# libmir/mir-optim

Measured on AMD Instinct MI355X. Metric: LM iterations/sec, higher is better.
Workload: dtype f64

## Files before the change

mir_optim_amd/csrc/workloads_device.h:

```cpp
#pragma once

#include <hip/hip_runtime.h>
#include <omp.h>

#include <cmath>
#include <cstddef>
#include <cstdint>
#include <cstdlib>
#include <type_traits>

namespace {


template <int N> __device__ inline int dpp_row_ror(int v) { return __builtin_amdgcn_update_dpp(0, v, 0x120 + N, 0xF, 0xF, false); }
template <int N> __device__ inline double dpp_row_ror(double v)
{
    return __hiloint2double(dpp_row_ror<N>(__double2hiint(v)), dpp_row_ror<N>(__double2loint(v)));
}
template <int N> __device__ inline float dpp_row_ror(float v) { return __int_as_float(dpp_row_ror<N>(__float_as_int(v))); }
template <typename T> __device__ inline T sum16(T v)
{
    v += dpp_row_ror<8>(v);
    v += dpp_row_ror<4>(v);
    v += dpp_row_ror<2>(v);
    v += dpp_row_ror<1>(v);
    return v;
}

template <int N, typename F, int I = 0> __device__ __forceinline__ void wl_static_for(F&& f)
{
    if constexpr (I < N) {
        f(std::integral_constant<int, I>{});
        wl_static_for<N, F, I + 1>(static_cast<F&&>(f));
    }
}

__device__ inline double lane_pair_swap(double v)
{
    const int lo = __builtin_amdgcn_mov_dpp(__double2loint(v), 0xB1, 0xF, 0xF, true);
    const int hi = __builtin_amdgcn_mov_dpp(__double2hiint(v), 0xB1, 0xF, 0xF, true);
    return __hiloint2double(hi, lo);
}

__device__ inline double dtanh(double x)
{
    const double ax = fabs(x);
    const double t = fmin(2.0 * ax, 40.0);
    const double kf = rint(t * 1.4426950408889634);
    double r = fma(kf, -6.93147180369123816490e-01, t);
    r = fma(kf, -1.90821492927058770002e-10, r);
    double p = 1.0 / 6227020800.0;
    p = fma(p, r, 1.0 / 479001600.0);
    p = fma(p, r, 1.0 / 39916800.0);
    p = fma(p, r, 1.0 / 3628800.0);
    p = fma(p, r, 1.0 / 362880.0);
    p = fma(p, r, 1.0 / 40320.0);
    p = fma(p, r, 1.0 / 5040.0);
    p = fma(p, r, 1.0 / 720.0);
    p = fma(p, r, 1.0 / 120.0);
    p = fma(p, r, 1.0 / 24.0);
    p = fma(p, r, 1.0 / 6.0);
    p = fma(p, r, 0.5);
    p = fma(p, r, 1.0);
    p = fma(p, r, 1.0);
    const double e = ldexp(p, (int)kf);
    const double d = e + 1.0;
    double q = __builtin_amdgcn_rcp(d);
    q = fma(fma(-d, q, 1.0), q, q);
    q = fma(fma(-d, q, 1.0), q, q);
    return copysign(fma(-2.0, q, 1.0), x);
}
__device__ inline float dtanh(float v) { return tanhf(v); }
__device__ inline double dexp(double v) { return exp(v); }
__device__ inline float dexp(float v) { return expf(v); }


}
```

mir_optim_amd/csrc/workloads_gemm.hip:

```cpp
#include "workloads_gemm.h"
#include "workloads_device.h"

namespace {

template <int NK>
__global__ __launch_bounds__(1024) void k_tanh_linear_batched(const double* __restrict__ A, const double* __restrict__ b,
                                                               const double* __restrict__ X, double* __restrict__ Y,
                                                               size_t m, int n, int P)
{
    using Acc = __attribute__((ext_vector_type(4))) double;
    constexpr int NPAD = 4 * NK;
    constexpr int PITCH = NPAD + 2;
    __shared__ __attribute__((aligned(16))) double tile[2][16 * PITCH];
    const int tid = threadIdx.x, lane = tid & 63, wave = tid >> 6;
    const int fr = lane & 15, fq = lane >> 4;

    for (int idx = tid; idx < 2 * 16 * PITCH; idx += 1024) (&tile[0][0])[idx] = 0.0;
    __syncthreads();

    const int ppr = n / 2;
    const bool has_piece = tid < 16 * ppr;
    const int prow = has_piece ? tid / ppr : 0, pcol = has_piece ? tid % ppr : 0;
    const size_t ntiles = (m + 15) / 16;

    for (int pbase = 0; pbase < P; pbase += 256) {
        const int pl = pbase + wave * 16 + fr;
        const bool pok = pl < P;
        const bool wave_active = pbase + wave * 16 < P;
        double xf[NK];
#pragma unroll
        for (int s = 0; s < NK; ++s) {
            const int col = 4 * s + fq;
            xf[s] = (pok && col < n) ? X[(size_t)pl * n + col] : 0.0;
        }
        double2 stage = make_double2(0.0, 0.0);
        auto gload = [&](size_t t) {
            const size_t row = t * 16 + prow;
            if (has_piece && row < m) stage = *reinterpret_cast<const double2*>(A + row * (size_t)n + 2 * pcol);
            else stage = make_double2(0.0, 0.0);
        };
        auto lstore = [&](int buf) {
            if (has_piece) *reinterpret_cast<double2*>(&tile[buf][prow * PITCH + 2 * pcol]) = stage;
        };
        size_t t = blockIdx.x;
        if (t < ntiles) { gload(t); lstore(0); }
        if (t + gridDim.x < ntiles) gload(t + gridDim.x);
        __syncthreads();
        int buf = 0;
        Acc prev = {0.0, 0.0, 0.0, 0.0};
        size_t tprev = ntiles;
        auto epilogue = [&](const Acc& acc, size_t tt) {
#pragma unroll
            for (int r = 0; r < 4; ++r) {
                const size_t row = tt * 16 + fq + 4 * r;
                if (pok && tt < ntiles && row < m) Y[(size_t)pl * m + row] = dtanh(acc[r]) - b[row];
            }
        };
        for (; t < ntiles; t += gridDim.x) {
            if (wave_active) {
                Acc acc = {0.0, 0.0, 0.0, 0.0};
                const double* tp = &tile[buf][fr * PITCH + fq];
#pragma unroll
                for (int s = 0; s < NK; ++s) acc = __builtin_amdgcn_mfma_f64_16x16x4f64(tp[4 * s], xf[s], acc, 0, 0, 0);
                epilogue(prev, tprev);
                prev = acc;
                tprev = t;
            }
            if (t + gridDim.x < ntiles) lstore(buf ^ 1);
            if (t + 2 * (size_t)gridDim.x < ntiles) gload(t + 2 * (size_t)gridDim.x);
            __syncthreads();
            buf ^= 1;
        }
        if (wave_active) epilogue(prev, tprev);
        __syncthreads();
    }
}


typedef __attribute__((address_space(3))) void* wl_lds_ptr;
typedef const __attribute__((address_space(1))) void* wl_gbl_ptr;

__device__ __forceinline__ constexpr int tlb_rho(int i) { return ((i >> 2) >> 1) * 8 + 2 * (i & 3) + ((i >> 2) & 1); }
__device__ __forceinline__ constexpr int tlb_sigma(int i) { return (i + 12) & 15; }

template <int NK> struct TlbCfg {
    static constexpr int N = 4 * NK;
    static constexpr int PPR = N / 2;
    static constexpr int TILES = NK <= 32 ? 2 : 1;
    static constexpr bool SELF = NK > 32;
    static constexpr int COMPUTE_WAVES = 8, LOADER_WAVES = SELF ? 0 : 2;
    static constexpr int CHUNK = 16 * COMPUTE_WAVES;
    static constexpr int ROWS = 16 * TILES;
    static constexpr int STAGE_BYTES = ROWS * N * 8;
    static constexpr int IPS = STAGE_BYTES / 1024;
    static constexpr int NS = 4, D = 2, NSB = 8;
    static constexpr int B_OFF = NS * STAGE_BYTES;
    static constexpr int LDS_BYTES = B_OFF + NSB * 256;
    static constexpr int THREADS = 64 * (COMPUTE_WAVES + LOADER_WAVES);
    static constexpr bool FORK = NK == 32;
    static constexpr int NPRE = NK / 2 - 1;
    static constexpr int PRE_STAGE = TILES * NPRE * 16 * 8;
    static constexpr int PRE_OFF = LDS_BYTES;
    static constexpr int VOTE_OFF = PRE_OFF + 2 * PRE_STAGE;
    static constexpr int FORK_LDS_BYTES = VOTE_OFF + 16;
};

template <int NK, int LOADER>
__device__ __forceinline__ void tlb_issue(const double* __restrict__ A, const double* __restrict__ b, size_t m,
                                          unsigned char* smem, int lane, size_t S, size_t f)
{
    using C = TlbCfg<NK>;
    constexpr int MYI = C::IPS / 2;
    const unsigned char* Ab = reinterpret_cast<const unsigned char*>(A);
    const unsigned char* bb = reinterpret_cast<const unsigned char*>(b);
    const size_t stage = blockIdx.x + (f % S) * (size_t)gridDim.x;
    const size_t row0 = stage * C::ROWS;
    unsigned char* slot = smem + (f % C::NS) * C::STAGE_BYTES;
#pragma unroll
    for (int k = 0; k < MYI; ++k) {
        const int ins = LOADER + 2 * k;
        const int g = ins * 64 + lane;
        const int R = g / C::PPR, sp = g % C::PPR;
        size_t row = row0 + (R & 16) + tlb_rho(R & 15);
        row = row < m ? row : m - 1;
        const int piece = sp ^ tlb_sigma(R & 15);
        __builtin_amdgcn_global_load_lds((wl_gbl_ptr)(Ab + (row * C::N + 2 * piece) * 8),
                                         (wl_lds_ptr)(slot + ins * 1024), 16, 0, 2 );
    }
    if constexpr (LOADER == 1) {
        size_t row = row0 + (lane >> 1);
        row = row < m ? row : m - 1;
        __builtin_amdgcn_global_load_lds((wl_gbl_ptr)(bb + row * 8 + (lane & 1) * 4),
                                         (wl_lds_ptr)(smem + C::B_OFF + (f % C::NSB) * 256), 4, 0, 0);
    }
}

template <int NK, int LOADER>
__device__ __forceinline__ void tlb_loader(const double* __restrict__ A, const double* __restrict__ b, size_t m,
                                           unsigned char* smem, int lane, size_t S, size_t F)
{
    using C = TlbCfg<NK>;
    constexpr int OPS = C::IPS / 2 + (LOADER == 1 ? 1 : 0);
    auto issue = [&](size_t f) { tlb_issue<NK, LOADER>(A, b, m, smem, lane, S, f); };
    const size_t pre = F < (size_t)C::D ? F : (size_t)C::D;
    for (size_t f = 0; f < pre; ++f) issue(f);
    for (size_t f = 0; f < F; ++f) {
        if (f + C::D < F) {
            issue(f + C::D);
            asm volatile("s_waitcnt vmcnt(%0)" ::"n"(C::D * OPS) : "memory");
        } else {
            asm volatile("s_waitcnt vmcnt(0)" ::: "memory");
        }
        __builtin_amdgcn_s_barrier();
    }
}

template <int NK, bool ALIGNED, int GROUP, bool RM = false, bool DIFF = false>
__device__ __forceinline__ void tlb_compute(const double* __restrict__ A, const double* __restrict__ b,
                                            const double* __restrict__ X, double* __restrict__ Y, size_t m, int P,
                                            unsigned char* smem, int lane, int wave, size_t S, int nchunks)
{
    using C = TlbCfg<NK>;
    using Acc = __attribute__((ext_vector_type(4))) double;
    const int fr = lane & 15, fq = lane >> 4;
    const int v = fq ^ tlb_sigma(fr);
    int laddr[4];
#pragma unroll
    for (int k = 0; k < 4; ++k) laddr[k] = fr * C::N * 8 + ((4 * k) ^ v) * 16;

    constexpr int MYI = C::SELF ? C::IPS / C::COMPUTE_WAVES : 1;
    [[maybe_unused]] int roff[MYI], soff[MYI];
    [[maybe_unused]] unsigned is_next = 0, slot_next = 0, bslot_next = 0;
    [[maybe_unused]] const size_t Ftot = S * (size_t)nchunks;
    [[maybe_unused]] size_t fissued = 0;
    const unsigned char* Ab = reinterpret_cast<const unsigned char*>(A);
    const unsigned char* bb = reinterpret_cast<const unsigned char*>(b);
    if constexpr (C::SELF) {
#pragma unroll
        for (int k = 0; k < MYI; ++k) {
            const int g = (wave + C::COMPUTE_WAVES * k) * 64 + lane;
            const int R = g / C::PPR, sp = g % C::PPR;
            roff[k] = (R & 16) + tlb_rho(R & 15);
            soff[k] = 2 * (sp ^ tlb_sigma(R & 15)) * 8;
        }
    }
    auto issue = [&]() {
        const size_t row0 = (blockIdx.x + (size_t)is_next * gridDim.x) * C::ROWS;
        unsigned char* slot = smem + slot_next * C::STAGE_BYTES;
#pragma unroll
        for (int k = 0; k < MYI; ++k) {
            size_t row = row0 + roff[k];
            row = row < m ? row : m - 1;
            __builtin_amdgcn_global_load_lds((wl_gbl_ptr)(Ab + row * (C::N * 8) + soff[k]),
                                             (wl_lds_ptr)(slot + (wave + C::COMPUTE_WAVES * k) * 1024), 16, 0, 2 );
        }
        if (wave == 0) {
            size_t row = row0 + (lane >> 1);
            row = row < m ? row : m - 1;
            __builtin_amdgcn_global_load_lds((wl_gbl_ptr)(bb + row * 8 + (lane & 1) * 4),
                                             (wl_lds_ptr)(smem + C::B_OFF + bslot_next * 256), 4, 0, 0);
        }
        is_next = is_next + 1 == (unsigned)S ? 0 : is_next + 1;
        slot_next = (slot_next + 1) % C::NS;
        bslot_next = (bslot_next + 1) % C::NSB;
        ++fissued;
    };
    auto advance = [&]() {
        if constexpr (C::SELF) {
            if (fissued < Ftot) {
                issue();
                if (wave == 0) asm volatile("s_waitcnt vmcnt(%0)" ::"n"(C::D * (MYI + 1)) : "memory");
                else asm volatile("s_waitcnt vmcnt(%0)" ::"n"(C::D * MYI) : "memory");
            } else {
                asm volatile("s_waitcnt vmcnt(0)" ::: "memory");
            }
        }
    };
    if constexpr (C::SELF) {
        for (int d = 0; d < C::D && fissued < Ftot; ++d) issue();
        advance();
    }

    size_t f = 0;
    for (int ch = 0; ch < nchunks; ++ch) {
        const bool wave_active = ch * C::CHUNK + wave * 16 < P;
        if (!wave_active) {
            for (size_t s = 0; s < S; ++s) {
                __builtin_amdgcn_s_barrier();
                ++f;
                if (f < Ftot) advance();
            }
            continue;
        }
        int pl = ch * C::CHUNK + wave * 16 + fr;
        pl = pl < P ? pl : P - 1;
        double xf[NK];
#pragma unroll
        for (int s = 0; s < NK; ++s) xf[s] = X[(size_t)pl * C::N + 8 * (s >> 1) + 2 * fq + (s & 1)];
        double* yp = DIFF ? Y + (pl >> 1) : (RM ? Y + pl : Y + (size_t)pl * m);
        const size_t ldr = DIFF ? (size_t)(P >> 1) : (RM ? (size_t)P : 1);

        auto mfma_stage = [&](size_t ff, Acc& acc0, Acc& acc1) {
            const unsigned char* slot = smem + (ff % C::NS) * C::STAGE_BYTES;
            acc0 = Acc{0, 0, 0, 0};
            acc1 = Acc{0, 0, 0, 0};
            if constexpr (C::TILES == 2) {
#pragma unroll
                for (int j = 0; j < NK / 2; ++j) {
                    const int off = laddr[j & 3] + (j >> 2) * 256;
                    const double2 a0 = *reinterpret_cast<const double2*>(slot + off);
                    const double2 a1 = *reinterpret_cast<const double2*>(slot + off + 16 * C::N * 8);
                    acc0 = __builtin_amdgcn_mfma_f64_16x16x4f64(a0.x, xf[2 * j], acc0, 0, 0, 0);
                    acc1 = __builtin_amdgcn_mfma_f64_16x16x4f64(a1.x, xf[2 * j], acc1, 0, 0, 0);
                    acc0 = __builtin_amdgcn_mfma_f64_16x16x4f64(a0.y, xf[2 * j + 1], acc0, 0, 0, 0);
                    acc1 = __builtin_amdgcn_mfma_f64_16x16x4f64(a1.y, xf[2 * j + 1], acc1, 0, 0, 0);
                }
            } else {
#pragma unroll
                for (int j = 0; j < NK / 2; j += 2) {
                    const double2 a0 = *reinterpret_cast<const double2*>(slot + laddr[j & 3] + (j >> 2) * 256);
                    const double2 a1 = *reinterpret_cast<const double2*>(slot + laddr[(j + 1) & 3] + ((j + 1) >> 2) * 256);
                    acc0 = __builtin_amdgcn_mfma_f64_16x16x4f64(a0.x, xf[2 * j], acc0, 0, 0, 0);
                    acc1 = __builtin_amdgcn_mfma_f64_16x16x4f64(a1.x, xf[2 * j + 2], acc1, 0, 0, 0);
                    acc0 = __builtin_amdgcn_mfma_f64_16x16x4f64(a0.y, xf[2 * j + 1], acc0, 0, 0, 0);
                    acc1 = __builtin_amdgcn_mfma_f64_16x16x4f64(a1.y, xf[2 * j + 3], acc1, 0, 0, 0);
                }
                acc0 += acc1;
            }
        };
        auto epilogue_tile = [&](const Acc& acc, size_t row0, const unsigned char* bslot, auto full_tag) {
            constexpr bool FULL = decltype(full_tag)::value;
            const double2 b0 = *reinterpret_cast<const double2*>(bslot + 16 * fq);
            const double2 b1 = *reinterpret_cast<const double2*>(bslot + 64 + 16 * fq);
            const double y0 = dtanh(acc[0]) - b0.x, y1 = dtanh(acc[1]) - b0.y;
            const double y2 = dtanh(acc[2]) - b1.x, y3 = dtanh(acc[3]) - b1.y;
            const size_t ra = row0 + 2 * fq, rb = row0 + 8 + 2 * fq;
            if constexpr (DIFF) {
                const double d0 = y0 - lane_pair_swap(y0), d1 = y1 - lane_pair_swap(y1);
                const double d2 = y2 - lane_pair_swap(y2), d3 = y3 - lane_pair_swap(y3);
                if ((fr & 1) == 0) {
                    if (FULL || ra < m) yp[ra * ldr] = d0;
                    if (FULL || ra + 1 < m) yp[(ra + 1) * ldr] = d1;
                    if (FULL || rb < m) yp[rb * ldr] = d2;
                    if (FULL || rb + 1 < m) yp[(rb + 1) * ldr] = d3;
                }
            } else if constexpr (RM) {
                if (FULL || ra < m) yp[ra * ldr] = y0;
                if (FULL || ra + 1 < m) yp[(ra + 1) * ldr] = y1;
                if (FULL || rb < m) yp[rb * ldr] = y2;
                if (FULL || rb + 1 < m) yp[(rb + 1) * ldr] = y3;
            } else if constexpr (FULL && ALIGNED) {
                *reinterpret_cast<double2*>(yp + ra) = make_double2(y0, y1);
                *reinterpret_cast<double2*>(yp + rb) = make_double2(y2, y3);
            } else if constexpr (FULL) {
                yp[ra] = y0;
                yp[ra + 1] = y1;
                yp[rb] = y2;
                yp[rb + 1] = y3;
            } else {
                if (ra < m) yp[ra] = y0;
                if (ra + 1 < m) yp[ra + 1] = y1;
                if (rb < m) yp[rb] = y2;
                if (rb + 1 < m) yp[rb + 1] = y3;
            }
        };
        auto epilogue = [&](const Acc& e0, const Acc& e1, size_t s, size_t ff, auto full_tag) {
            const size_t row0 = (blockIdx.x + s * (size_t)gridDim.x) * C::ROWS;
            const unsigned char* bs = smem + C::B_OFF + (ff % C::NSB) * 256;
            epilogue_tile(e0, row0, bs, full_tag);
            __builtin_amdgcn_sched_barrier(0);
            if constexpr (C::TILES == 2) {
                epilogue_tile(e1, row0 + 16, bs + 128, full_tag);
                __builtin_amdgcn_sched_barrier(0);
            }
        };
        Acc acc0, acc1;
        if constexpr (GROUP == 0) {
            for (size_t s = 0; s + 1 < S; ++s, ++f) {
                __builtin_amdgcn_s_barrier();
                mfma_stage(f, acc0, acc1);
                advance();
                epilogue(acc0, acc1, s, f, std::true_type{});
            }
            __builtin_amdgcn_s_barrier();
            mfma_stage(f, acc0, acc1);
            if (f + 1 < Ftot) advance();
            epilogue(acc0, acc1, S - 1, f, std::false_type{});
            ++f;
        } else {
            __builtin_amdgcn_s_barrier();
            mfma_stage(f, acc0, acc1);
            ++f;
            if (f < Ftot) advance();
            for (size_t s = 1; s < S; ++s, ++f) {
                __builtin_amdgcn_s_barrier();
                epilogue(acc0, acc1, s - 1, f - 1, std::true_type{});
                mfma_stage(f, acc0, acc1);
                if (f + 1 < Ftot) advance();
            }
            epilogue(acc0, acc1, S - 1, f - 1, std::false_type{});
        }
    }
}

template <int NK, int GROUP>
__device__ __forceinline__ void tlb_compute_once(const double* __restrict__ X, double* __restrict__ D, size_t m,
                                                 unsigned char* smem, int lane, int wave, size_t S)
{
    using C = TlbCfg<NK>;
    using Acc = __attribute__((ext_vector_type(4))) double;
    constexpr int N = C::N, P = 2 * C::N;
    constexpr int NCH = (P + C::CHUNK - 1) / C::CHUNK;
    const int fr = lane & 15, fq = lane >> 4;
    const int v = fq ^ tlb_sigma(fr);
    int laddr[4];
#pragma unroll
    for (int k = 0; k < 4; ++k) laddr[k] = fr * N * 8 + ((4 * k) ^ v) * 16;

    double xb[NK];
#pragma unroll
    for (int s = 0; s < NK; ++s) {
        const int k = 8 * (s >> 1) + 2 * fq + (s & 1);
        xb[s] = X[(size_t)((2 * k + 2) % P) * N + k];
    }
    bool act[NCH], hit[NCH];
    int sstar[NCH];
    double xs[NCH];
    double* dp[NCH];
#pragma unroll
    for (int c = 0; c < NCH; ++c) {
        act[c] = c * C::CHUNK + wave * 16 < P;
        int pl = c * C::CHUNK + wave * 16 + fr;
        pl = pl < P ? pl : P - 1;
        const int j = pl >> 1;
        hit[c] = fq == ((j >> 1) & 3);
        sstar[c] = 2 * (j >> 3) + (j & 1);
        xs[c] = X[(size_t)pl * N + j];
        dp[c] = D + j;
    }
    constexpr size_t ldr = N;

    auto mfma_stage = [&](size_t st, auto cc, Acc& acc0, Acc& acc1) {
        constexpr int c = decltype(cc)::value;
        const unsigned char* slot = smem + (st % C::NS) * C::STAGE_BYTES;
        acc0 = Acc{0, 0, 0, 0};
        acc1 = Acc{0, 0, 0, 0};
        auto xop = [&](int s) { return (hit[c] && sstar[c] == s) ? xs[c] : xb[s]; };
        if constexpr (C::TILES == 2) {
#pragma unroll
            for (int j = 0; j < NK / 2; ++j) {
                const int off = laddr[j & 3] + (j >> 2) * 256;
                const double2 a0 = *reinterpret_cast<const double2*>(slot + off);
                const double2 a1 = *reinterpret_cast<const double2*>(slot + off + 16 * N * 8);
                const double x0 = xop(2 * j), x1 = xop(2 * j + 1);
                acc0 = __builtin_amdgcn_mfma_f64_16x16x4f64(a0.x, x0, acc0, 0, 0, 0);
                acc1 = __builtin_amdgcn_mfma_f64_16x16x4f64(a1.x, x0, acc1, 0, 0, 0);
                acc0 = __builtin_amdgcn_mfma_f64_16x16x4f64(a0.y, x1, acc0, 0, 0, 0);
                acc1 = __builtin_amdgcn_mfma_f64_16x16x4f64(a1.y, x1, acc1, 0, 0, 0);
            }
        } else {
#pragma unroll
            for (int j = 0; j < NK / 2; j += 2) {
                const double2 a0 = *reinterpret_cast<const double2*>(slot + laddr[j & 3] + (j >> 2) * 256);
                const double2 a1 = *reinterpret_cast<const double2*>(slot + laddr[(j + 1) & 3] + ((j + 1) >> 2) * 256);
                acc0 = __builtin_amdgcn_mfma_f64_16x16x4f64(a0.x, xop(2 * j), acc0, 0, 0, 0);
                acc1 = __builtin_amdgcn_mfma_f64_16x16x4f64(a1.x, xop(2 * j + 2), acc1, 0, 0, 0);
                acc0 = __builtin_amdgcn_mfma_f64_16x16x4f64(a0.y, xop(2 * j + 1), acc0, 0, 0, 0);
                acc1 = __builtin_amdgcn_mfma_f64_16x16x4f64(a1.y, xop(2 * j + 3), acc1, 0, 0, 0);
            }
            acc0 += acc1;
        }
    };
    auto epilogue_tile = [&](const Acc& acc, size_t row0, const unsigned char* bslot, double* yp, bool full) {
        const double2 b0 = *reinterpret_cast<const double2*>(bslot + 16 * fq);
        const double2 b1 = *reinterpret_cast<const double2*>(bslot + 64 + 16 * fq);
        const double y0 = dtanh(acc[0]) - b0.x, y1 = dtanh(acc[1]) - b0.y;
        const double y2 = dtanh(acc[2]) - b1.x, y3 = dtanh(acc[3]) - b1.y;
        const double d0 = y0 - lane_pair_swap(y0), d1 = y1 - lane_pair_swap(y1);
        const double d2 = y2 - lane_pair_swap(y2), d3 = y3 - lane_pair_swap(y3);
        const size_t ra = row0 + 2 * fq, rb = row0 + 8 + 2 * fq;
        if ((fr & 1) == 0) {
            if (full || ra < m) yp[ra * ldr] = d0;
            if (full || ra + 1 < m) yp[(ra + 1) * ldr] = d1;
            if (full || rb < m) yp[rb * ldr] = d2;
            if (full || rb + 1 < m) yp[(rb + 1) * ldr] = d3;
        }
    };
    auto epilogue = [&](const Acc& e0, const Acc& e1, size_t st, auto cc) {
        constexpr int c = decltype(cc)::value;
        const size_t row0 = (blockIdx.x + st * (size_t)gridDim.x) * C::ROWS;
        const unsigned char* bs = smem + C::B_OFF + (st % C::NSB) * 256;
        const bool full = st + 1 < S;
        epilogue_tile(e0, row0, bs, dp[c], full);
        __builtin_amdgcn_sched_barrier(0);
        if constexpr (C::TILES == 2) {
            epilogue_tile(e1, row0 + 16, bs + 128, dp[c], full);
            __builtin_amdgcn_sched_barrier(0);
        }
    };
    Acc acc0, acc1;
    if constexpr (GROUP == 0) {
        for (size_t st = 0; st < S; ++st) {
            __builtin_amdgcn_s_barrier();
            wl_static_for<NCH>([&](auto cc) {
                if (act[decltype(cc)::value]) {
                    mfma_stage(st, cc, acc0, acc1);
                    epilogue(acc0, acc1, st, cc);
                }
            });
        }
    } else {
        for (size_t st = 0; st < S; ++st) {
            wl_static_for<NCH>([&](auto cc) {
                constexpr int c = decltype(cc)::value;
                if constexpr (c == 0) {
                    __builtin_amdgcn_s_barrier();
                    if (st > 0) {
                        wl_static_for<NCH>([&](auto pp) {
                            constexpr int pc = decltype(pp)::value;
                            constexpr bool last = pc == NCH - 1;
                            if (act[pc] && (last || !act[pc + (last ? 0 : 1)])) epilogue(acc0, acc1, st - 1, pp);
                        });
                    }
                    if (act[0]) mfma_stage(st, cc, acc0, acc1);
                } else {
                    if (act[c]) {
                        epilogue(acc0, acc1, st, std::integral_constant<int, c - 1>{});
                        mfma_stage(st, cc, acc0, acc1);
                    }
                }
            });
        }
        if (S > 0) {
            wl_static_for<NCH>([&](auto pp) {
                constexpr int pc = decltype(pp)::value;
                constexpr bool last = pc == NCH - 1;
                if (act[pc] && (last || !act[pc + (last ? 0 : 1)])) epilogue(acc0, acc1, S - 1, pp);
            });
        }
    }
}


template <int NK>
__device__ __forceinline__ bool tlb_fork_vote(const double* __restrict__ X, unsigned char* smem, int lane, int wave)
{
    using C = TlbCfg<NK>;
    constexpr int N = C::N, P = 2 * N;
    volatile int* vote = reinterpret_cast<volatile int*>(smem + C::VOTE_OFF);
    if (threadIdx.x == 0) *vote = 0;
    __syncthreads();
    if (wave < C::COMPUTE_WAVES) {
        const int fr = lane & 15, fq = lane >> 4;
        const int s0 = 2 * (wave ^ 2), s1 = 2 * (2 * C::COMPUTE_WAVES - 1 - wave);
        const unsigned long long* xr = reinterpret_cast<const unsigned long long*>(X);
        const unsigned long long* x0 = xr + (size_t)(8 * s0 + fr) * N;
        const unsigned long long* x1 = xr + (size_t)(8 * s1 + fr) * N;
        bool bad = false;
#pragma unroll
        for (int s = 0; s < NK - 2; ++s) {
            const int k = 8 * (s >> 1) + 2 * fq + (s & 1);
            const unsigned long long xb = xr[(size_t)((2 * k + 2) % P) * N + k];
            const unsigned long long a = x0[k], c = x1[k];
            bad |= (s < s0) & (a != xb);
            bad |= (s < s1) & (c != xb);
        }
        if (bad) *vote = 1;
    }
    __syncthreads();
    return *vote == 0;
}

template <int NK, int LOADER>
__device__ __forceinline__ void tlb_fork_loader(const double* __restrict__ A, const double* __restrict__ b,
                                                const double* __restrict__ X, size_t m, unsigned char* smem, int lane, size_t S)
{
    using C = TlbCfg<NK>;
    using Acc = __attribute__((ext_vector_type(4))) double;
    constexpr int N = C::N, P = 2 * N;
    constexpr int OPS = C::IPS / 2 + (LOADER == 1 ? 1 : 0);
    const int fr = lane & 15, fq = lane >> 4;
    const int v = fq ^ tlb_sigma(fr);
    int laddr[4];
#pragma unroll
    for (int k = 0; k < 4; ++k) laddr[k] = LOADER * 16 * N * 8 + fr * N * 8 + ((4 * k) ^ v) * 16;
    double xb[2 * C::NPRE];
#pragma unroll
    for (int s = 0; s < 2 * C::NPRE; ++s) {
        const int k = 8 * (s >> 1) + 2 * fq + (s & 1);
        xb[s] = X[(size_t)((2 * k + 2) % P) * N + k];
    }
    auto issue = [&](size_t f) { tlb_issue<NK, LOADER>(A, b, m, smem, lane, S, f); };
    for (size_t f = 0; f < S && f < (size_t)C::D; ++f) issue(f);
    for (size_t f = 0; f < S; ++f) {
        if (f + 1 < S) asm volatile("s_waitcnt vmcnt(%0)" ::"n"(OPS) : "memory");
        else asm volatile("s_waitcnt vmcnt(0)" ::: "memory");
        __builtin_amdgcn_s_barrier();
        asm volatile("" ::: "memory");
        if (f + C::D < S) issue(f + C::D);
        const unsigned char* slot = smem + (f % C::NS) * C::STAGE_BYTES;
        double* pre = reinterpret_cast<double*>(smem + C::PRE_OFF + (f & 1) * C::PRE_STAGE) + LOADER * C::NPRE * 16 + 4 * fq;
        Acc acc = {0.0, 0.0, 0.0, 0.0};
#pragma unroll
        for (int j = 0; j < C::NPRE; ++j) {
            const double2 a = *reinterpret_cast<const double2*>(slot + laddr[j & 3] + (j >> 2) * 256);
            acc = __builtin_amdgcn_mfma_f64_16x16x4f64(a.x, xb[2 * j], acc, 0, 0, 0);
            acc = __builtin_amdgcn_mfma_f64_16x16x4f64(a.y, xb[2 * j + 1], acc, 0, 0, 0);
            if (fr == 0) {
                *reinterpret_cast<double2*>(pre + 16 * j) = make_double2(acc[0], acc[1]);
                *reinterpret_cast<double2*>(pre + 16 * j + 2) = make_double2(acc[2], acc[3]);
            }
        }
        asm volatile("s_waitcnt lgkmcnt(0)" ::: "memory");
    }
    __builtin_amdgcn_s_barrier();
}

template <int NK, int W>
__device__ __forceinline__ void tlb_fork_compute(const double* __restrict__ X, double* __restrict__ D, size_t m,
                                                 unsigned char* smem, int lane, size_t S)
{
    using C = TlbCfg<NK>;
    using Acc = __attribute__((ext_vector_type(4))) double;
    constexpr int N = C::N;
    constexpr int GA = W ^ 2, GC = 2 * C::COMPUTE_WAVES - 1 - W;
    constexpr int SA = 2 * GA, SC = 2 * GC;
    constexpr int GROUP = W < C::COMPUTE_WAVES / 2 ? 0 : 1;
    const int fr = lane & 15, fq = lane >> 4;
    const int v = fq ^ tlb_sigma(fr);
    int laddr[4];
#pragma unroll
    for (int k = 0; k < 4; ++k) laddr[k] = fr * N * 8 + ((4 * k) ^ v) * 16;
    const int pa = 16 * GA + fr, pc = 16 * GC + fr;
    double xa[NK - SA], xc[NK - SC];
#pragma unroll
    for (int s = SA; s < NK; ++s) xa[s - SA] = X[(size_t)pa * N + 8 * (s >> 1) + 2 * fq + (s & 1)];
#pragma unroll
    for (int s = SC; s < NK; ++s) xc[s - SC] = X[(size_t)pc * N + 8 * (s >> 1) + 2 * fq + (s & 1)];
    double* const da = D + (pa >> 1);
    double* const dc = D + (pc >> 1);
    constexpr size_t ldr = N;

    auto mfma_stage = [&](size_t f, Acc (&acc)[4]) {
        const unsigned char* slot = smem + (f % C::NS) * C::STAGE_BYTES;
        const double* pre = reinterpret_cast<const double*>(smem + C::PRE_OFF + (f & 1) * C::PRE_STAGE) + 4 * fq;
        auto prefix = [&](int t, int s) {
            if (s == 0) return Acc{0.0, 0.0, 0.0, 0.0};
            const double* p = pre + (t * C::NPRE + s / 2 - 1) * 16;
            const double2 lo = *reinterpret_cast<const double2*>(p), hi = *reinterpret_cast<const double2*>(p + 2);
            return Acc{lo.x, lo.y, hi.x, hi.y};
        };
        acc[0] = prefix(0, SA);
        acc[1] = prefix(1, SA);
        acc[2] = prefix(0, SC);
        acc[3] = prefix(1, SC);
        wl_static_for<NK / 2 - GA>([&](auto jj) {
            constexpr int j = GA + decltype(jj)::value;
            const int off = laddr[j & 3] + (j >> 2) * 256;
            const double2 a0 = *reinterpret_cast<const double2*>(slot + off);
            const double2 a1 = *reinterpret_cast<const double2*>(slot + off + 16 * N * 8);
            acc[0] = __builtin_amdgcn_mfma_f64_16x16x4f64(a0.x, xa[2 * j - SA], acc[0], 0, 0, 0);
            acc[1] = __builtin_amdgcn_mfma_f64_16x16x4f64(a1.x, xa[2 * j - SA], acc[1], 0, 0, 0);
            if constexpr (j >= GC) {
                acc[2] = __builtin_amdgcn_mfma_f64_16x16x4f64(a0.x, xc[2 * j - SC], acc[2], 0, 0, 0);
                acc[3] = __builtin_amdgcn_mfma_f64_16x16x4f64(a1.x, xc[2 * j - SC], acc[3], 0, 0, 0);
            }
            acc[0] = __builtin_amdgcn_mfma_f64_16x16x4f64(a0.y, xa[2 * j + 1 - SA], acc[0], 0, 0, 0);
            acc[1] = __builtin_amdgcn_mfma_f64_16x16x4f64(a1.y, xa[2 * j + 1 - SA], acc[1], 0, 0, 0);
            if constexpr (j >= GC) {
                acc[2] = __builtin_amdgcn_mfma_f64_16x16x4f64(a0.y, xc[2 * j + 1 - SC], acc[2], 0, 0, 0);
                acc[3] = __builtin_amdgcn_mfma_f64_16x16x4f64(a1.y, xc[2 * j + 1 - SC], acc[3], 0, 0, 0);
            }
        });
    };
    auto epilogue_tile = [&](const Acc& acc, size_t row0, const unsigned char* bslot, double* yp, bool full) {
        const double2 b0 = *reinterpret_cast<const double2*>(bslot + 16 * fq);
        const double2 b1 = *reinterpret_cast<const double2*>(bslot + 64 + 16 * fq);
        const double y0 = dtanh(acc[0]) - b0.x, y1 = dtanh(acc[1]) - b0.y;
        const double y2 = dtanh(acc[2]) - b1.x, y3 = dtanh(acc[3]) - b1.y;
        const double d0 = y0 - lane_pair_swap(y0), d1 = y1 - lane_pair_swap(y1);
        const double d2 = y2 - lane_pair_swap(y2), d3 = y3 - lane_pair_swap(y3);
        const size_t ra = row0 + 2 * fq, rb = row0 + 8 + 2 * fq;
        if ((fr & 1) == 0) {
            if (full || ra < m) yp[ra * ldr] = d0;
            if (full || ra + 1 < m) yp[(ra + 1) * ldr] = d1;
            if (full || rb < m) yp[rb * ldr] = d2;
            if (full || rb + 1 < m) yp[(rb + 1) * ldr] = d3;
        }
    };
    auto epilogue = [&](const Acc (&acc)[4], size_t f) {
        const size_t row0 = (blockIdx.x + f * (size_t)gridDim.x) * C::ROWS;
        const unsigned char* bs = smem + C::B_OFF + (f % C::NSB) * 256;
        const bool full = f + 1 < S;
        epilogue_tile(acc[0], row0, bs, da, full);
        __builtin_amdgcn_sched_barrier(0);
        epilogue_tile(acc[1], row0 + 16, bs + 128, da, full);
        __builtin_amdgcn_sched_barrier(0);
        epilogue_tile(acc[2], row0, bs, dc, full);
        __builtin_amdgcn_sched_barrier(0);
        epilogue_tile(acc[3], row0 + 16, bs + 128, dc, full);
        __builtin_amdgcn_sched_barrier(0);
    };
    auto barrier = [] {
        asm volatile("" ::: "memory");
        __builtin_amdgcn_s_barrier();
        asm volatile("" ::: "memory");
    };
    Acc acc[4];
    barrier();
    if constexpr (GROUP == 0) {
        for (size_t f = 0; f < S; ++f) {
            barrier();
            mfma_stage(f, acc);
            epilogue(acc, f);
        }
    } else {
        barrier();
        mfma_stage(0, acc);
        for (size_t f = 1; f < S; ++f) {
            barrier();
            epilogue(acc, f - 1);
            mfma_stage(f, acc);
        }
        epilogue(acc, S - 1);
    }
}

template <int NK, bool RM = false, bool DIFF = false>
__global__ __launch_bounds__(TlbCfg<NK>::THREADS) void k_tanh_linear_batched_dma(const double* __restrict__ A,
                                                                                  const double* __restrict__ b,
                                                                                  const double* __restrict__ X,
                                                                                  double* __restrict__ Y, size_t m, int P,
                                                                                  int mode)
{
    using C = TlbCfg<NK>;
    extern __shared__ __attribute__((aligned(16))) unsigned char tlb_smem[];
    const int lane = threadIdx.x & 63;
    const int wave = __builtin_amdgcn_readfirstlane(threadIdx.x >> 6);
    const size_t Stot = (m + C::ROWS - 1) / C::ROWS;
    const size_t S = blockIdx.x < Stot ? (Stot - blockIdx.x + gridDim.x - 1) / gridDim.x : 0;
    const int nchunks = (P + C::CHUNK - 1) / C::CHUNK;
    const bool once = DIFF && mode == 1 && NK <= 32 && P == 2 * C::N;
    const size_t F = once ? S : S * (size_t)nchunks;
    if (S == 0) return;
    if constexpr (DIFF && C::FORK) {
        if (mode == 2 && P == 2 * C::N && tlb_fork_vote<NK>(X, tlb_smem, lane, wave)) {
            if (wave == C::COMPUTE_WAVES) tlb_fork_loader<NK, 0>(A, b, X, m, tlb_smem, lane, S);
            else if (wave == C::COMPUTE_WAVES + 1) tlb_fork_loader<NK, 1>(A, b, X, m, tlb_smem, lane, S);
            else wl_static_for<C::COMPUTE_WAVES>([&](auto ww) {
                if (wave == decltype(ww)::value) tlb_fork_compute<NK, decltype(ww)::value>(X, Y, m, tlb_smem, lane, S);
            });
            return;
        }
    }
    if (!C::SELF && wave == C::COMPUTE_WAVES) tlb_loader<NK, 0>(A, b, m, tlb_smem, lane, S, F);
    else if (!C::SELF && wave == C::COMPUTE_WAVES + 1) tlb_loader<NK, 1>(A, b, m, tlb_smem, lane, S, F);
    else if (DIFF && once) {
        if constexpr (DIFF) {
            if (wave < 4) tlb_compute_once<NK, 0>(X, Y, m, tlb_smem, lane, wave, S);
            else tlb_compute_once<NK, 1>(X, Y, m, tlb_smem, lane, wave, S);
        }
    } else {
        if constexpr (RM) {
            if (wave < 4) tlb_compute<NK, false, 0, true, DIFF>(A, b, X, Y, m, P, tlb_smem, lane, wave, S, nchunks);
            else tlb_compute<NK, false, 1, true, DIFF>(A, b, X, Y, m, P, tlb_smem, lane, wave, S, nchunks);
        } else {
            const bool aligned = ((m & 1) == 0) && ((reinterpret_cast<uintptr_t>(Y) & 15) == 0);
            if (wave < 4) {
                if (aligned) tlb_compute<NK, true, 0>(A, b, X, Y, m, P, tlb_smem, lane, wave, S, nchunks);
                else tlb_compute<NK, false, 0>(A, b, X, Y, m, P, tlb_smem, lane, wave, S, nchunks);
            } else {
                if (aligned) tlb_compute<NK, true, 1>(A, b, X, Y, m, P, tlb_smem, lane, wave, S, nchunks);
                else tlb_compute<NK, false, 1>(A, b, X, Y, m, P, tlb_smem, lane, wave, S, nchunks);
            }
        }
    }
}

template <int NK, bool RM = false, bool DIFF = false>
bool launch_tlb_dma(const double* A, const double* b, const double* X, double* Y, size_t m, int P, hipStream_t s, int mode = 0)
{
    using C = TlbCfg<NK>;
    constexpr int lds = DIFF && C::FORK ? C::FORK_LDS_BYTES : C::LDS_BYTES;
    static bool attr_ok = [] {
        return hipFuncSetAttribute(reinterpret_cast<const void*>(k_tanh_linear_batched_dma<NK, RM, DIFF>),
                                   hipFuncAttributeMaxDynamicSharedMemorySize, lds) == hipSuccess;
    }();
    if (!attr_ok) return false;
    const size_t Stot = (m + C::ROWS - 1) / C::ROWS;
    const unsigned grid = (unsigned)(Stot < 256 ? Stot : 256);
    hipLaunchKernelGGL((k_tanh_linear_batched_dma<NK, RM, DIFF>), dim3(grid), dim3(C::THREADS), lds, s, A, b, X, Y, m, P, mode);
    return true;
}

__global__ __launch_bounds__(256) void k_tanh_linear_batched_rm_generic(const double* __restrict__ A, const double* __restrict__ b,
                                                                        const double* __restrict__ X, double* __restrict__ Y,
                                                                        size_t m, int n, int P)
{
    const size_t total = m * (size_t)P;
    for (size_t e = (size_t)blockIdx.x * blockDim.x + threadIdx.x; e < total; e += (size_t)gridDim.x * blockDim.x) {
        const size_t i = e / P;
        const int k = (int)(e % P);
        const double* a = A + i * (size_t)n;
        const double* x = X + (size_t)k * n;
        double s0 = 0;
        for (int j = 0; j < n; ++j) s0 += a[j] * x[j];
        Y[e] = dtanh(s0) - b[i];
    }
}

__global__ __launch_bounds__(256) void k_tanh_linear_batched_diff_generic(const double* __restrict__ A, const double* __restrict__ b,
                                                                          const double* __restrict__ X, double* __restrict__ D,
                                                                          size_t m, int n, int P)
{
    const int nc = P / 2;
    const size_t total = m * (size_t)nc;
    for (size_t e = (size_t)blockIdx.x * blockDim.x + threadIdx.x; e < total; e += (size_t)gridDim.x * blockDim.x) {
        const size_t i = e / nc;
        const int j = (int)(e % nc);
        const double* a = A + i * (size_t)n;
        const double* xp = X + (size_t)(2 * j) * n;
        const double* xm = xp + n;
        double sp = 0, sm = 0;
        for (int k = 0; k < n; ++k) { sp += a[k] * xp[k]; sm += a[k] * xm[k]; }
        const double yp = dtanh(sp) - b[i], ym = dtanh(sm) - b[i];
        D[e] = yp - ym;
    }
}

template <int OUT>
__global__ __launch_bounds__(256) void k_tanh_linear_batched_wide(const double* __restrict__ A, const double* __restrict__ b,
                                                                    const double* __restrict__ X, double* __restrict__ Y,
                                                                    size_t m, int n, int P)
{
    constexpr int RT = 4;
    using Acc = __attribute__((ext_vector_type(4))) double;
    const int lane = threadIdx.x & 63, wave = threadIdx.x >> 6;
    const int fr = lane & 15, fq = lane >> 4;
    const size_t ntiles = (m + 16 * RT - 1) / (16 * RT);
    const int ngroups = (P + 63) / 64;
    const int npairs = n / 8;
    for (size_t t = blockIdx.x; t < ntiles; t += gridDim.x) {
        const double2* __restrict__ ap[RT];
        double bv[RT][4];
#pragma unroll
        for (int rt = 0; rt < RT; ++rt) {
            const size_t r0 = (t * RT + rt) * 16;
            const size_t arow = r0 + fr < m ? r0 + fr : m - 1;
            ap[rt] = reinterpret_cast<const double2*>(A + arow * (size_t)n) + fq;
#pragma unroll
            for (int r = 0; r < 4; ++r) { const size_t row = r0 + fq + 4 * r; bv[rt][r] = b[row < m ? row : m - 1]; }
        }
        for (int g = wave; g < ngroups; g += 4) {
            const double2* __restrict__ xp[4];
#pragma unroll
            for (int u = 0; u < 4; ++u) {
                int pt = 64 * g + 16 * u + fr;
                pt = pt < P ? pt : P - 1;
                xp[u] = reinterpret_cast<const double2*>(X + (size_t)pt * n) + fq;
            }
            Acc acc[RT][4];
#pragma unroll
            for (int rt = 0; rt < RT; ++rt)
#pragma unroll
                for (int u = 0; u < 4; ++u) acc[rt][u] = Acc{0, 0, 0, 0};
#pragma unroll 2
            for (int j = 0; j < npairs; ++j) {
                double2 a[RT], x[4];
#pragma unroll
                for (int rt = 0; rt < RT; ++rt) a[rt] = ap[rt][4 * j];
#pragma unroll
                for (int u = 0; u < 4; ++u) x[u] = xp[u][4 * j];
#pragma unroll
                for (int rt = 0; rt < RT; ++rt)
#pragma unroll
                    for (int u = 0; u < 4; ++u) {
                        acc[rt][u] = __builtin_amdgcn_mfma_f64_16x16x4f64(a[rt].x, x[u].x, acc[rt][u], 0, 0, 0);
                        acc[rt][u] = __builtin_amdgcn_mfma_f64_16x16x4f64(a[rt].y, x[u].y, acc[rt][u], 0, 0, 0);
                    }
            }
#pragma unroll
            for (int rt = 0; rt < RT; ++rt)
#pragma unroll
                for (int u = 0; u < 4; ++u) {
                    const int pt = 64 * g + 16 * u + fr;
#pragma unroll
                    for (int r = 0; r < 4; ++r) {
                        const size_t row = (t * RT + rt) * 16 + fq + 4 * r;
                        const double y = dtanh(acc[rt][u][r]) - bv[rt][r];
                        if constexpr (OUT == 1) {
                            const double d = y - lane_pair_swap(y);
                            if ((fr & 1) == 0 && pt < P && row < m) Y[row * (size_t)(P >> 1) + (pt >> 1)] = d;
                        } else if constexpr (OUT == 0) {
                            if (pt < P && row < m) Y[row * (size_t)P + pt] = y;
                        } else {
                            if (pt < P && row < m) Y[(size_t)pt * m + row] = y;
                        }
                    }
                }
        }
    }
}

}

void launch_tanh_linear_batched_diff(const double* A, const double* b, const double* X, double* D, size_t m, int n, int P,
                                     hipStream_t s, int read_a_once, bool dense)
{
    if (m >= 32 && P % 16 == 0) {
        const int mode = read_a_once ? 1 : dense ? 0 : 2;
        if (n == 256 && launch_tlb_dma<64, true, true>(A, b, X, D, m, P, s, mode)) return;
        if (n == 128 && launch_tlb_dma<32, true, true>(A, b, X, D, m, P, s, mode)) return;
        if (n == 64 && launch_tlb_dma<16, true, true>(A, b, X, D, m, P, s, mode)) return;
        if (n == 32 && launch_tlb_dma<8, true, true>(A, b, X, D, m, P, s, mode)) return;
    }
    if (n > 256 && n % 8 == 0 && P % 2 == 0 && m > 0) {
        const size_t nt = (m + 63) / 64;
        hipLaunchKernelGGL(k_tanh_linear_batched_wide<1>, dim3((unsigned)(nt < 256 * 8 ? nt : 256 * 8)), dim3(256), 0, s, A, b, X, D, m, n, P);
        return;
    }
    size_t blocks = (m * (size_t)(P / 2) + 255) / 256;
    if (blocks > 256 * 16) blocks = 256 * 16;
    hipLaunchKernelGGL(k_tanh_linear_batched_diff_generic, dim3((unsigned)(blocks ? blocks : 1)), dim3(256), 0, s, A, b, X, D, m, n, P);
}

void launch_tanh_linear_batched_rm(const double* A, const double* b, const double* X, double* Y, size_t m, int n, int P,
                                   hipStream_t s)
{
    if (m >= 32) {
        if (n == 256 && launch_tlb_dma<64, true>(A, b, X, Y, m, P, s)) return;
        if (n == 128 && launch_tlb_dma<32, true>(A, b, X, Y, m, P, s)) return;
        if (n == 64 && launch_tlb_dma<16, true>(A, b, X, Y, m, P, s)) return;
        if (n == 32 && launch_tlb_dma<8, true>(A, b, X, Y, m, P, s)) return;
    }
    if (n > 256 && n % 8 == 0 && m > 0) {
        const size_t nt = (m + 63) / 64;
        hipLaunchKernelGGL(k_tanh_linear_batched_wide<0>, dim3((unsigned)(nt < 256 * 8 ? nt : 256 * 8)), dim3(256), 0, s, A, b, X, Y, m, n, P);
        return;
    }
    size_t blocks = (m * (size_t)P + 255) / 256;
    if (blocks > 256 * 16) blocks = 256 * 16;
    hipLaunchKernelGGL(k_tanh_linear_batched_rm_generic, dim3((unsigned)(blocks ? blocks : 1)), dim3(256), 0, s, A, b, X, Y, m, n, P);
}

bool launch_tanh_linear_batched(const double* A, const double* b, const double* X, double* Y, size_t m, int n, int P,
                                hipStream_t s)
{
    if (n == 256 && m >= 32 && launch_tlb_dma<64>(A, b, X, Y, m, P, s)) return true;
    if (n > 256 && n % 8 == 0 && m > 0) {
        const size_t nt = (m + 63) / 64;
        hipLaunchKernelGGL(k_tanh_linear_batched_wide<2>, dim3((unsigned)(nt < 256 * 8 ? nt : 256 * 8)), dim3(256), 0, s, A, b, X, Y, m, n, P);
        return true;
    }
    if (n % 2 != 0 || n > 128 || n < 4) return false;
    if (m >= 32) {
        if (n == 128 && launch_tlb_dma<32>(A, b, X, Y, m, P, s)) return true;
        if (n == 64 && launch_tlb_dma<16>(A, b, X, Y, m, P, s)) return true;
        if (n == 32 && launch_tlb_dma<8>(A, b, X, Y, m, P, s)) return true;
    }
    const size_t ntiles = (m + 15) / 16;
    unsigned grid = (unsigned)(ntiles < 256 ? ntiles : 256);
    if (n <= 16) hipLaunchKernelGGL(k_tanh_linear_batched<4>, dim3(grid), dim3(1024), 0, s, A, b, X, Y, m, n, P);
    else if (n <= 32) hipLaunchKernelGGL(k_tanh_linear_batched<8>, dim3(grid), dim3(1024), 0, s, A, b, X, Y, m, n, P);
    else if (n <= 64) hipLaunchKernelGGL(k_tanh_linear_batched<16>, dim3(grid), dim3(1024), 0, s, A, b, X, Y, m, n, P);
    else hipLaunchKernelGGL(k_tanh_linear_batched<32>, dim3(grid), dim3(1024), 0, s, A, b, X, Y, m, n, P);
    return true;
}
```

Before: 1130.

## Rework fork-compute epilogue with buffer stores, lane-balanced pair diffs, uniform schedule

The epilogue of the fork compute path now has both lanes of each pair store one difference. Previously only even lanes wrote four values each. Stores go through raw buffer resources sized to the tile, so hardware bounds clamping handles out-of-range rows, and a compile-time FULL tag removes the per-store bound checks in steady-state iterations. It also drops the staggered two-group schedule, where half the waves overlapped the epilogue with the next MFMA stage, in favour of one uniform loop. That may lose overlap between waves, and the stored layout relies on the new offset arithmetic being correct.

Measured after the change: 1133 (median of 6 runs). About the same (+0.3%).

```diff
diff --git a/mir_optim_amd/csrc/workloads_device.h b/mir_optim_amd/csrc/workloads_device.h
--- a/mir_optim_amd/csrc/workloads_device.h
+++ b/mir_optim_amd/csrc/workloads_device.h
@@ -42,6 +42,13 @@
     return __hiloint2double(hi, lo);
 }
 
+__device__ inline double wl_pair_diff(double y0, double y1, bool odd)
+{
+    const double r = lane_pair_swap(odd ? y0 : y1);
+    const double u = odd ? r : y0, w = odd ? y1 : r;
+    return u - w;
+}
+
 __device__ inline double dtanh(double x)
 {
     const double ax = fabs(x);
diff --git a/mir_optim_amd/csrc/workloads_gemm.hip b/mir_optim_amd/csrc/workloads_gemm.hip
--- a/mir_optim_amd/csrc/workloads_gemm.hip
+++ b/mir_optim_amd/csrc/workloads_gemm.hip
@@ -79,6 +79,16 @@
 
 typedef __attribute__((address_space(3))) void* wl_lds_ptr;
 typedef const __attribute__((address_space(1))) void* wl_gbl_ptr;
+
+__device__ __forceinline__ __amdgpu_buffer_rsrc_t tlb_rsrc(double* base, unsigned bytes)
+{
+    return __builtin_amdgcn_make_buffer_rsrc(base, (short)0, (int)bytes, 0x00020000);
+}
+__device__ __forceinline__ void tlb_store(__amdgpu_buffer_rsrc_t rs, unsigned voff, unsigned soff, double v)
+{
+    using U2 = __attribute__((ext_vector_type(2))) unsigned;
+    __builtin_amdgcn_raw_buffer_store_b64(__builtin_bit_cast(U2, v), rs, (int)voff, (int)soff, 0);
+}
 
 __device__ __forceinline__ constexpr int tlb_rho(int i) { return ((i >> 2) >> 1) * 8 + 2 * (i & 3) + ((i >> 2) & 1); }
 __device__ __forceinline__ constexpr int tlb_sigma(int i) { return (i + 12) & 15; }
@@ -565,7 +575,6 @@
     constexpr int N = C::N;
     constexpr int GA = W ^ 2, GC = 2 * C::COMPUTE_WAVES - 1 - W;
     constexpr int SA = 2 * GA, SC = 2 * GC;
-    constexpr int GROUP = W < C::COMPUTE_WAVES / 2 ? 0 : 1;
     const int fr = lane & 15, fq = lane >> 4;
     const int v = fq ^ tlb_sigma(fr);
     int laddr[4];
@@ -577,9 +586,9 @@
     for (int s = SA; s < NK; ++s) xa[s - SA] = X[(size_t)pa * N + 8 * (s >> 1) + 2 * fq + (s & 1)];
 #pragma unroll
     for (int s = SC; s < NK; ++s) xc[s - SC] = X[(size_t)pc * N + 8 * (s >> 1) + 2 * fq + (s & 1)];
-    double* const da = D + (pa >> 1);
-    double* const dc = D + (pc >> 1);
-    constexpr size_t ldr = N;
+    const bool odd = fr & 1;
+    const unsigned lrow = 2 * fq + odd;
+    const unsigned oa = (lrow * N + (pa >> 1)) * 8, oc = (lrow * N + (pc >> 1)) * 8;
 
     auto mfma_stage = [&](size_t f, Acc (&acc)[4]) {
         const unsigned char* slot = smem + (f % C::NS) * C::STAGE_BYTES;
@@ -613,32 +622,32 @@
             }
         });
     };
-    auto epilogue_tile = [&](const Acc& acc, size_t row0, const unsigned char* bslot, double* yp, bool full) {
-        const double2 b0 = *reinterpret_cast<const double2*>(bslot + 16 * fq);
-        const double2 b1 = *reinterpret_cast<const double2*>(bslot + 64 + 16 * fq);
+    auto epilogue_tile = [&](const Acc& acc, int t, __amdgpu_buffer_rsrc_t rs, unsigned o, const double2& b0, const double2& b1,
+                             size_t rem, auto full_tag) {
+        constexpr bool FULL = decltype(full_tag)::value;
         const double y0 = dtanh(acc[0]) - b0.x, y1 = dtanh(acc[1]) - b0.y;
         const double y2 = dtanh(acc[2]) - b1.x, y3 = dtanh(acc[3]) - b1.y;
-        const double d0 = y0 - lane_pair_swap(y0), d1 = y1 - lane_pair_swap(y1);
-        const double d2 = y2 - lane_pair_swap(y2), d3 = y3 - lane_pair_swap(y3);
-        const size_t ra = row0 + 2 * fq, rb = row0 + 8 + 2 * fq;
-        if ((fr & 1) == 0) {
-            if (full || ra < m) yp[ra * ldr] = d0;
-            if (full || ra + 1 < m) yp[(ra + 1) * ldr] = d1;
-            if (full || rb < m) yp[rb * ldr] = d2;
-            if (full || rb + 1 < m) yp[(rb + 1) * ldr] = d3;
-        }
+        const double da = wl_pair_diff(y0, y1, odd), db = wl_pair_diff(y2, y3, odd);
+        const unsigned r = 16 * t + lrow;
+        if (FULL || r < rem) tlb_store(rs, o, 16 * t * N * 8, da);
+        if (FULL || r + 8 < rem) tlb_store(rs, o, (16 * t + 8) * N * 8, db);
     };
-    auto epilogue = [&](const Acc (&acc)[4], size_t f) {
+    auto epilogue = [&](const Acc (&acc)[4], size_t f, auto full_tag) {
         const size_t row0 = (blockIdx.x + f * (size_t)gridDim.x) * C::ROWS;
         const unsigned char* bs = smem + C::B_OFF + (f % C::NSB) * 256;
-        const bool full = f + 1 < S;
-        epilogue_tile(acc[0], row0, bs, da, full);
+        const size_t rem = m - row0;
+        const __amdgpu_buffer_rsrc_t rs = tlb_rsrc(D + row0 * N, (unsigned)(rem < C::ROWS ? rem : C::ROWS) * N * 8);
+        double2 b0 = *reinterpret_cast<const double2*>(bs + 16 * fq);
+        double2 b1 = *reinterpret_cast<const double2*>(bs + 64 + 16 * fq);
+        epilogue_tile(acc[0], 0, rs, oa, b0, b1, rem, full_tag);
         __builtin_amdgcn_sched_barrier(0);
-        epilogue_tile(acc[1], row0 + 16, bs + 128, da, full);
+        epilogue_tile(acc[2], 0, rs, oc, b0, b1, rem, full_tag);
         __builtin_amdgcn_sched_barrier(0);
-        epilogue_tile(acc[2], row0, bs, dc, full);
+        b0 = *reinterpret_cast<const double2*>(bs + 128 + 16 * fq);
+        b1 = *reinterpret_cast<const double2*>(bs + 192 + 16 * fq);
+        epilogue_tile(acc[1], 1, rs, oa, b0, b1, rem, full_tag);
         __builtin_amdgcn_sched_barrier(0);
-        epilogue_tile(acc[3], row0 + 16, bs + 128, dc, full);
+        epilogue_tile(acc[3], 1, rs, oc, b0, b1, rem, full_tag);
         __builtin_amdgcn_sched_barrier(0);
     };
     auto barrier = [] {
@@ -648,22 +657,14 @@
     };
     Acc acc[4];
     barrier();
-    if constexpr (GROUP == 0) {
-        for (size_t f = 0; f < S; ++f) {
-            barrier();
-            mfma_stage(f, acc);
-            epilogue(acc, f);
-        }
-    } else {
+    for (size_t f = 0; f + 1 < S; ++f) {
         barrier();
-        mfma_stage(0, acc);
-        for (size_t f = 1; f < S; ++f) {
-            barrier();
-            epilogue(acc, f - 1);
-            mfma_stage(f, acc);
-        }
-        epilogue(acc, S - 1);
-    }
+        mfma_stage(f, acc);
+        epilogue(acc, f, std::true_type{});
+    }
+    barrier();
+    mfma_stage(S - 1, acc);
+    epilogue(acc, S - 1, std::false_type{});
 }
 
 template <int NK, bool RM = false, bool DIFF = false>
```
